# flydog-sdr/FlyDog_SDR_GPS

Hardware: AMD Instinct MI355X
Metric: IQ Msamples/s ingested (waterfall + GPS acq); value = GPS acq, BASELINE configs[1] (higher is better)
Workload: dtype f32

## Files before the change

### flydog_sdr_gps_amd/csrc/kg_acq.hip

```cpp
#include "kg_common.h"
#include "kg_fft.h"

#include <math.h>
#include <stdlib.h>
#include <vector>

#define SUB      4096
#define NTAPS    31
#define DECIM    4


enum { SRC_BITS = 0, SRC_IQ16 = 1, SRC_CHIPS = 2 };

__constant__ float c_hb_even[16] = {
    -0.010233f,  0.010668f, -0.016324f,  0.024377f, -0.036482f,  0.056990f, -0.101993f,
     0.316926f,  0.316926f, -0.101993f,  0.056990f, -0.036482f,  0.024377f, -0.016324f,
     0.010668f, -0.010233f,
};
#define HB_CENTRE 0.500009f

KG_DEV float bipolar(int bit) { return bit ? -1.0f : 1.0f; }

template <int SRC>
KG_DEV cf acq_source(const void *__restrict__ src, int i, int nvalid, int nchips, int boc)
{
    if (i >= nvalid) return cf{0.f, 0.f};
    if constexpr (SRC == SRC_BITS) {
        const uint8_t *p = (const uint8_t *) src;
        const int bit = (p[i >> 3] >> (i & 7)) & 1;
        const int ph = i & 3;
        const int ls = ph < 2, lc = (ph == 0) | (ph == 3);
        return cf{bipolar(bit ^ ls), bipolar(bit ^ lc)};
    } else if constexpr (SRC == SRC_IQ16) {
        const short2 v = ((const short2 *) src)[i];
// ... 134 lines not shown
            if (ii >= 512 - halo) {
                const int jj = (j + 1) & 7;
                kg_st(&o[(jj >> 1) * row + 2 * (ii - 512 + halo) + (jj & 1)], fq[q]);
            }
        }
    }
}

struct acq_red { float p; int i; float s; int pad; };

#define ACQ_CLAIM_STRIDE 32
#define ACQ_LDS_BYTES (2 * SUB * sizeof(float2) + 4 * sizeof(acq_red) + 16)

struct acq_pair_desc {
    int data_off;
    int code_off;
    int limit;
    int out;
};

struct acq_cell_desc { int data_off, code_off, dop, limit, out; };

struct acq_walk {
    int npairs;
    int ndop, dop_lo;
};

template <int P, bool STAMPS = false>
__global__ __launch_bounds__(256, 2) void acq_correlate_kernel(
    const float2 *__restrict__ data,
    const float2 *__restrict__ code,
    const float2 *__restrict__ tab4096, const float2 *__restrict__ tabN,
    const float2 *__restrict__ comb,
    const float2 *__restrict__ quart,
    const acq_pair_desc *__restrict__ pairs,
    int *__restrict__ claim,
    acq_walk walk,
    int halo,
    kg_acq_cell *__restrict__ cells,
    unsigned long long *__restrict__ stamps = nullptr)
{
    static_assert(P == 4 || P == 16, "N = 16384 or 65536");
    constexpr int LOGP = P == 4 ? 2 : 4;
    extern __shared__ __attribute__((aligned(16))) float2 smem[];
    float2 *tileA = smem, *tileB = smem + SUB;
    acq_red *red = (acq_red *) (smem + 2 * SUB);
    volatile int *red_claim = (volatile int *) (red + 4);
    const int t = threadIdx.x;
    unsigned long long *st = (STAMPS && t == 0 && blockIdx.x == 8) ? stamps : nullptr;
    if (STAMPS && st) { st[0] = __builtin_amdgcn_s_memtime(); st[1] = __builtin_amdgcn_s_memrealtime(); }
    unsigned long long *wgt = (STAMPS && t == 0) ? stamps + 512 + 4 * blockIdx.x : nullptr;
    int wg_cells = 0;
    if (STAMPS && wgt) {
        wgt[0] = __builtin_amdgcn_s_memrealtime();
        wgt[2] = (unsigned long long) __builtin_amdgcn_s_getreg((20 << 0) | (0 << 6) | (31 << 11));
    }

    kg_tw4096 tw;
    kg_tw4096_load(tw, tab4096, t);
    cf wb[3], wa[3];
#pragma unroll
    for (int i = 1; i < 4; i++) { wb[i - 1] = kg_ld(&tabN[t * i]); wa[i - 1] = kg_ld(&tabN[(4 * t * i) & (P * SUB - 1)]); }
    (void) wa;
    auto sel3 = [](const cf (&w)[3], int i) { return i == 1 ? w[0] : (i == 2 ? w[1] : w[2]); };

    const int xcd = blockIdx.x & 7, slot = blockIdx.x >> 3, nslots = gridDim.x >> 3;
    const int gpairs = (walk.npairs - xcd + 7) >> 3;
    const bool spread = walk.npairs < 8;
    const int ndop = walk.ndop, ncell = spread ? (walk.npairs * ndop - xcd + 7) >> 3 : gpairs * ndop;

    typedef unsigned u4 __attribute__((ext_vector_type(4)));
    const int rowb_c = 2 * (256 + 2 * halo) * (int) sizeof(float2);
    const int plane_c = 8 * 2 * (256 + 2 * halo);
    cf d[16], c[16];
    struct acq_rsrc { __amdgpu_buffer_rsrc_t drs, crs; int dvo, cvo; };
    auto fetch_prepare = [&](int data_off, int code_off, int dop, int k2) {
        const int s = k2 - dop;
        const int q0 = s >> LOGP;
        acq_rsrc r;
        r.drs = __builtin_amdgcn_make_buffer_rsrc(
            (void *) (data + data_off + k2 * SUB), 0, SUB * (int) sizeof(float2), 0x00020000);
        r.crs = __builtin_amdgcn_make_buffer_rsrc(
            (void *) (code + code_off + (s & (P - 1)) * plane_c), 0, plane_c * (int) sizeof(float2), 0x00020000);
        r.dvo = t * 16; r.cvo = (t + q0 + halo) * 16;
        return r;
    };
    auto fetch_row = [&](const acq_rsrc &r, int i) {
        const u4 dv = __builtin_amdgcn_raw_buffer_load_b128(r.drs, r.dvo, i * 4096, 0);
        const u4 cv = __builtin_amdgcn_raw_buffer_load_b128(r.crs, r.cvo, i * rowb_c, 0);
        d[2 * i] = cf{__uint_as_float(dv[0]), __uint_as_float(dv[1])};
        d[2 * i + 1] = cf{__uint_as_float(dv[2]), __uint_as_float(dv[3])};
        c[2 * i] = cf{__uint_as_float(cv[0]), __uint_as_float(cv[1])};
        c[2 * i + 1] = cf{__uint_as_float(cv[2]), __uint_as_float(cv[3])};
    };
    auto fetch_drow = [&](const acq_rsrc &r, int i) {
        const u4 dv = __builtin_amdgcn_raw_buffer_load_b128(r.drs, r.dvo, i * 4096, 0);
        d[2 * i] = cf{__uint_as_float(dv[0]), __uint_as_float(dv[1])};
        d[2 * i + 1] = cf{__uint_as_float(dv[2]), __uint_as_float(dv[3])};
    };
    auto fetch_crow = [&](const acq_rsrc &r, int i) {
        const u4 cv = __builtin_amdgcn_raw_buffer_load_b128(r.crs, r.cvo, i * rowb_c, 0);
        c[2 * i] = cf{__uint_as_float(cv[0]), __uint_as_float(cv[1])};
        c[2 * i + 1] = cf{__uint_as_float(cv[2]), __uint_as_float(cv[3])};
    };
    auto fetch = [&](int data_off, int code_off, int dop, int k2) {
        const acq_rsrc r = fetch_prepare(data_off, code_off, dop, k2);
#pragma unroll
        for (int i = 0; i < 8; i++) fetch_row(r, i);
    };
    auto describe = [&](int idx) {
        const int cell = spread ? (idx << 3) + xcd : idx;
        const int pg = cell / ndop, di = cell - pg * ndop;
        const acq_pair_desc pd = pairs[spread ? pg : (pg << 3) + xcd];
        return acq_cell_desc{pd.data_off, pd.code_off, walk.dop_lo + di, pd.limit, pd.out + di};
    };

    int cur_idx = slot, nxt_idx = slot + nslots;
    if (cur_idx >= ncell) return;
    acq_cell_desc cur = describe(cur_idx);
    fetch(cur.data_off, cur.code_off, cur.dop, 0);

    int st_item = 0;
    for (;;) {
        const bool more = nxt_idx < ncell;
        const acq_cell_desc nxt = describe(more ? nxt_idx : cur_idx);
        int claimed = 0;
        if (t == 0) claimed = __hip_atomic_fetch_add(&claim[xcd * ACQ_CLAIM_STRIDE], 1, __ATOMIC_RELAXED, __HIP_MEMORY_SCOPE_AGENT);
        cf acc[16];
        cf yprev[16], pbase = cf{0.f, 0.f}, pg[3], pG[3];
        auto accumulate = [&](const cf (&yv)[16], int kp, cf bs, const cf (&g)[3], const cf (&G)[3]) {
            if (kp == 0) {
#pragma unroll
                for (int m = 0; m < 16; m++) acc[m] = yv[m];
                return;
            }
            cf B1, B2, B3;
            kg_cmul1x3s(B1, B2, B3, bs, G[0], G[1], G[2]);
#pragma unroll
            for (int a = 0; a < 4; a++) {
                const cf Ba = a == 0 ? bs : (a == 1 ? B1 : (a == 2 ? B2 : B3));
                const cf C0 = Ba;
                cf C1, C2, C3;
                kg_cmul1x3s(C1, C2, C3, Ba, g[0], g[1], g[2]);
                kg_cmac4v(acc[4 * a], acc[4 * a + 1], acc[4 * a + 2], acc[4 * a + 3],
                          yv[4 * a], yv[4 * a + 1], yv[4 * a + 2], yv[4 * a + 3], C0, C1, C2, C3);
            }
        };
        auto accumulate_fenced = [&](int kp) { kg_pin(); accumulate(yprev, kp, pbase, pg, pG); kg_pin(); };
        const int tl = t & 15, th = t >> 4;
        const int rd = t ^ (th & 15);
#pragma unroll 1
        for (int k2 = 0; k2 < P; k2++) {
            unsigned long long *sti = (STAMPS && st && st_item < 24) ? st + 16 + 16 * st_item : nullptr;
            KG_STAMP(STAMPS, sti, 8);
            cf base;
            if constexpr (P == 4) base = sel3(wb, k2);
            else {
                const int ka = k2 >> 2, kb = k2 & 3;
                const cf A = sel3(wa, ka), Bv = sel3(wb, kb);
                base = ka == 0 ? Bv : (kb == 0 ? A : kg_cmul(A, Bv));
            }
            cf x[16], y[16];
            const bool same = k2 < P - 1;
            const acq_rsrc nr = fetch_prepare(same ? cur.data_off : nxt.data_off, same ? cur.code_off : nxt.code_off,
                                              same ? cur.dop : nxt.dop, (k2 + 1) & (P - 1));
            KG_STAMP(STAMPS, sti, 9);
            KG_STAMP(STAMPS, sti, 10);
            kg_cc_radix16_h<+1>(c, d, y, [&](int s) {
                kg_pin();
                if (s < 4) {
                    fetch_drow(nr, 2 * s); fetch_drow(nr, 2 * s + 1);
                } else {
#pragma unroll
                    for (int m = s - 4; m < 16; m += 4) kg_st_tile(&tileA[16 * t + (m ^ tl)], y[m]);
                }
                kg_pin();
            });
            KG_STAMP(STAMPS, sti, 0);
            KG_STAMP(STAMPS, sti, 1);
            __syncthreads();
            KG_STAMP(STAMPS, sti, 2);
#pragma unroll
            for (int j = 0; j < 16; j++) x[j] = kg_ld_tile(&tileA[rd + 256 * j]);
            if (k2 > 0) accumulate_fenced(k2 - 1);
            if (STAMPS) asm volatile("s_waitcnt lgkmcnt(0)" ::: "memory");
            KG_STAMP(STAMPS, sti, 3);
            kg_tw_radix16_h<+1>(x, y, tw.p1, [&](int s) {
                if (s >= 4) {
                    kg_pin();
#pragma unroll
                    for (int m = s - 4; m < 16; m += 4) kg_st_tile(&tileB[t + 16 * (15 * th + m)], y[m]);
                    kg_pin();
                }
            });
            KG_STAMP(STAMPS, sti, 4);
            __syncthreads();
            KG_STAMP(STAMPS, sti, 5);
            cf g[3], G[3];
#pragma unroll
            for (int i = 0; i < 3; i++) { g[i] = kg_ld(&comb[8 * k2 + i]); G[i] = kg_ld(&comb[8 * k2 + 3 + i]); }
#pragma unroll
            for (int j = 0; j < 16; j++) x[j] = kg_ld_tile(&tileB[t + 256 * j]);
            if (STAMPS) asm volatile("s_waitcnt lgkmcnt(0)" ::: "memory");
            KG_STAMP(STAMPS, sti, 6);
            kg_tw_radix16_h<+1>(x, yprev, tw.p2, [&](int s) {
                if (s < 4) { kg_pin(); fetch_crow(nr, 2 * s); fetch_crow(nr, 2 * s + 1); kg_pin(); }
            });
            pbase = base;
#pragma unroll
            for (int i = 0; i < 3; i++) { pg[i] = g[i]; pG[i] = G[i]; }
            KG_STAMP(STAMPS, sti, 7);
            KG_STAMP(STAMPS, sti, 11);
            if (STAMPS) st_item++;
        }
        accumulate(yprev, P - 1, pbase, pg, pG);

        const int limit = cur.limit, full_rows = limit >> 8;
        float bp = 0.f, sum = 0.f;
        int bi = 0;
        if constexpr (P == 4) {
            float pw[16];
#pragma unroll
            for (int m = 0; m < 16; m++) {
                const cf sq = acc[m] * acc[m];
                pw[m] = sq.x + sq.y;
                if (m >= full_rows) {
                    asm volatile("");
                    pw[m] = (t + 256 * m < limit) ? pw[m] : 0.f;
                }
            }
            cf s2 = cf{0.f, 0.f};
#pragma unroll
            for (int m = 0; m < 16; m += 2) s2 = s2 + cf{pw[m], pw[m + 1]};
            sum = s2.x + s2.y;
#pragma unroll
            for (int m = 0; m < 16; m += 2) bp = __builtin_fmaxf(bp, __builtin_fmaxf(pw[m], pw[m + 1]));
            unsigned qm[2] = {0, 0};
#pragma unroll
            for (int m = 7; m >= 0; m -= 2) {
                unsigned long long k0, k1, k2, k3;
                asm("v_cmp_eq_f32_e64 %2, %6, %10\n\tv_cmp_eq_f32_e64 %3, %7, %10\n\t"
                    "v_cmp_eq_f32_e64 %4, %8, %10\n\tv_cmp_eq_f32_e64 %5, %9, %10\n\t"
                    "v_addc_co_u32_e64 %0, %2, %0, %0, %2\n\tv_addc_co_u32_e64 %1, %3, %1, %1, %3\n\t"
                    "v_addc_co_u32_e64 %0, %4, %0, %0, %4\n\tv_addc_co_u32_e64 %1, %5, %1, %1, %5"
                    : "+v"(qm[0]), "+v"(qm[1]), "=&s"(k0), "=&s"(k1), "=&s"(k2), "=&s"(k3)
                    : "v"(pw[m]), "v"(pw[m + 8]), "v"(pw[m - 1]), "v"(pw[m + 7]), "v"(bp));
            }
            const unsigned rowmask = qm[0] | (qm[1] << 8);
// ... 459 lines not shown
    const int t = blockIdx.x * blockDim.x + threadIdx.x;
    if (t >= P * H) return;
    const int k2 = t % P, k1 = t / P;
    const float2 v = src ? src[(size_t) k2 * plane_len(H, layout_src) + plane_pos(k1, 0, H, layout_src)] : make_float2(0.f, 0.f);
    const int T = layout_dst == 0 ? 256 : 512, J = SUB / T;
    dst[(size_t) k2 * plane_len(H, layout_dst) + plane_pos(k1 + T * (J - 1), T, H, layout_dst)] = v;
}

static void to_planes(const float *nat, std::vector<float2> &pl, int P, int H, int layout)
{
    const size_t plane = plane_len(H, layout);
    const int T = layout == 0 ? 256 : 512, J = SUB / T;
    pl.assign(spec_len(P, H), make_float2(0.f, 0.f));
    for (int k = 0; k < P * SUB; k++) {
        const float2 v = make_float2(nat[2 * k], nat[2 * k + 1]);
        const int k1 = k / P, t = k1 & (T - 1), j = k1 / T;
        float2 *p = pl.data() + (size_t) (k % P) * plane;
        p[plane_pos(k1, 0, H, layout)] = v;
        if (t < H) p[plane_pos(t + T * ((j - 1) & (J - 1)), T, H, layout)] = v;
        if (t >= T - H) p[plane_pos(t + T * ((j + 1) & (J - 1)), -T, H, layout)] = v;
    }
}
static void from_planes(const std::vector<float2> &pl, float *nat, int P, int H, int layout)
{
    const size_t plane = plane_len(H, layout);
    for (int k = 0; k < P * SUB; k++) {
        const float2 v = pl[(size_t) (k % P) * plane + plane_pos(k / P, 0, H, layout)];
        nat[2 * k] = v.x; nat[2 * k + 1] = v.y;
    }
}

static float2 unit_root(long k, long n)
{
    k %= n;
    if (k < 0) k += n;
    if (k == 0) return make_float2(1.f, 0.f);
    if (4 * k == n) return make_float2(0.f, 1.f);
    if (2 * k == n) return make_float2(-1.f, 0.f);
    if (4 * k == 3 * n) return make_float2(0.f, -1.f);
    const double a = 2.0 * M_PI * (double) k / (double) n;
    return make_float2((float) cos(a), (float) sin(a));
}

template <int SRC>
static int launch_frontend(kg_acq *a, hipStream_t st, const uint8_t *d_src, size_t stride, int nbatch,
                           int nvalid, int nchips, int boc, float2 *d_td, float2 *d_scratch,
                           float2 *d_planes, float2 *d_planes_b, size_t planes_stride, int halo)
{
    kg_ctx *c = a->ctx;
    hipLaunchKernelGGL(acq_frontend_kernel<SRC>, dim3(a->fft_len / FE_TILE, nbatch), dim3(256), 0,
                       st, d_src, stride, nvalid, nchips, boc, d_td, a->fft_len);
    KG_HIP(hipGetLastError());
    hipLaunchKernelGGL(acq_fft_sub_kernel<false>, dim3(a->P, nbatch), dim3(256), 2 * SUB * sizeof(float2),
                       st, (const float2 *) d_td, d_scratch, (const float2 *) c->d_tab4096, a->P,
                       (unsigned long long *) nullptr);
    KG_HIP(hipGetLastError());
    if (a->P == 4)
        hipLaunchKernelGGL(acq_fft_combine_kernel<4>, dim3(SUB / 256, nbatch), dim3(256), 0, st,
                           (const float2 *) d_scratch, d_planes, d_planes_b, planes_stride,
                           (const float2 *) a->d_tabN, halo);
    else
        hipLaunchKernelGGL(acq_fft_combine_kernel<16>, dim3(SUB / 256, nbatch), dim3(256), 0, st,
                           (const float2 *) d_scratch, d_planes, d_planes_b, planes_stride,
                           (const float2 *) a->d_tabN, halo);
    KG_HIP(hipGetLastError());
    return KG_OK;
}

static int acq_init(kg_acq *a)
{
    kg_ctx *ctx = a->ctx;
    const int max_sats = a->max_sats, max_blocks = a->max_blocks, N = a->fft_len, P = a->P;
    {
        const int m = (a->dop_hi > -a->dop_lo ? a->dop_hi : -a->dop_lo);
        a->halo = (m + P - 1) / P + 2;
        a->code_len = spec_len(P, a->halo);
    }
    a->limits.assign(max_sats, 0); a->code_set.assign(max_sats, 0); a->code_layout.assign(max_sats, 0);
    a->last_first = a->last_nblocks = a->last_nsats = a->np1 = a->np4 = a->table_nblocks = 0;
    a->d_pairs1 = a->d_pairs4 = nullptr; a->pairs_seq = 0;
    a->in_stride = (size_t) a->nsamples * 4;
    const size_t spec = sizeof(float2) * N;
    if (N == 16384) { a->d_tabN = ctx->d_tab16384; a->own_tabN = false; }
    else {
        std::vector<float2> h(N);
        for (int k = 0; k < N; k++) h[k] = unit_root(k, N);
        KG_HIP(hipMalloc((void **) &a->d_tabN, spec));
        a->own_tabN = true;
        KG_HIP(hipMemcpy(a->d_tabN, h.data(), spec, hipMemcpyHostToDevice));
    }
    {
        const long R = N / 256;
        std::vector<float2> comb(P * 8, make_float2(1.f, 0.f)), quart(P * 4);
        static const int mult[6] = {1, 2, 3, 4, 8, 12};
        for (int k2 = 0; k2 < P; k2++) {
            for (int i = 0; i < 6; i++) comb[8 * k2 + i] = unit_root((long) mult[i] * k2, R);
            for (int q = 0; q < 4; q++) quart[4 * k2 + q] = unit_root((long) q * k2, P);
        }
        KG_HIP(hipMalloc((void **) &a->d_comb, sizeof(float2) * comb.size()));
        KG_HIP(hipMalloc((void **) &a->d_quart, sizeof(float2) * quart.size()));
        KG_HIP(hipMemcpy(a->d_comb, comb.data(), sizeof(float2) * comb.size(), hipMemcpyHostToDevice));
        KG_HIP(hipMemcpy(a->d_quart, quart.data(), sizeof(float2) * quart.size(), hipMemcpyHostToDevice));
        std::vector<float2> comb8(P * 4);
        for (int k2 = 0; k2 < P; k2++)
            for (int k = 0; k < 4; k++) comb8[4 * k2 + k] = unit_root((long) (k + 1) * k2, N / 512);
        KG_HIP(hipMalloc((void **) &a->d_comb8, sizeof(float2) * comb8.size()));
        KG_HIP(hipMemcpy(a->d_comb8, comb8.data(), sizeof(float2) * comb8.size(), hipMemcpyHostToDevice));
    }
    KG_HIP(hipMalloc((void **) &a->d_code, sizeof(float2) * a->code_len * max_sats));
    KG_HIP(hipMalloc((void **) &a->d_data, spec * max_blocks));
    KG_HIP(hipMalloc((void **) &a->d_td, spec * max_blocks));
    KG_HIP(hipMalloc((void **) &a->d_td_code, spec));
    KG_HIP(hipMalloc((void **) &a->d_fsub, spec * max_blocks));
    KG_HIP(hipMalloc((void **) &a->d_fsub_code, spec));
    KG_HIP(hipMalloc((void **) &a->d_in, a->in_stride * max_blocks));
    for (int k = 0; k < 4; k++) {
        KG_HIP(hipHostMalloc((void **) &a->h_pin[k], a->in_stride, hipHostMallocDefault));
        KG_HIP(hipEventCreateWithFlags(&a->ev_pin[k], hipEventDisableTiming));
    }
    KG_HIP(hipEventCreateWithFlags(&a->ev_batch, hipEventDisableTiming));
    KG_HIP(hipEventCreateWithFlags(&a->ev_in_free, hipEventDisableTiming));
    { const int rc_ = kg_stream_get(ctx->device, &a->cstream); if (rc_) return rc_; }
    KG_HIP(hipMalloc((void **) &a->d_chips, 8192));
    KG_HIP(hipMalloc((void **) &a->d_cells, sizeof(kg_acq_cell) * (size_t) max_blocks * max_sats * a->ndop));
    KG_HIP(hipMalloc((void **) &a->d_results, sizeof(kg_acq_result) * (size_t) max_blocks * max_sats));
    KG_HIP(hipMalloc((void **) &a->d_claim, sizeof(int) * 16 * ACQ_CLAIM_STRIDE));
    KG_HIP(hipMemset(a->d_claim, 0, sizeof(int) * 16 * ACQ_CLAIM_STRIDE));
    {
        const char *e = kg_tuning_env("KIWIGPU_ACQ_FRONT_STREAM");
        if (e && e[0] == '1') {
            { const int rc_ = kg_stream_get(ctx->device, &a->fstream); if (rc_) return rc_; }
// ... 393 lines not shown
    KG_HIP(hipStreamSynchronize(a->fstream));
    return KG_OK;
}

int kg_acq_get_data_fft(kg_acq *a, int block, float *data_fft)
{
    int rc = check_block(a, block, data_fft, "kg_acq_get_data_fft");
    if (rc) return rc;
    return get_planes(a, a->d_data + (size_t) block * a->fft_len, data_fft, 0, 0);
}

int kg_acq_get_data_td(kg_acq *a, int block, float *td)
{
    int rc = check_block(a, block, td, "kg_acq_get_data_td");
    if (rc) return rc;
    KG_HIP(hipStreamSynchronize(a->fstream));
    KG_HIP(hipMemcpyAsync(td, a->d_td + (size_t) block * a->fft_len, sizeof(float2) * a->fft_len,
                          hipMemcpyDeviceToHost, a->ctx->stream));
    KG_HIP(hipStreamSynchronize(a->ctx->stream));
    return KG_OK;
}

}

template <int P, bool STAMPS>
static void launch_correlate(kg_acq *a, hipStream_t st, int first, const acq_pair_desc *d_pairs, int npairs,
                             unsigned long long *d_stamps)
{
    const int grid = a->grid1;
    const acq_walk w = {npairs, a->ndop, a->dop_lo};
    hipLaunchKernelGGL((acq_correlate_kernel<P, STAMPS>), dim3(grid), dim3(256), ACQ_LDS_BYTES, st,
                       (const float2 *) (a->d_data + (size_t) first * a->fft_len), (const float2 *) a->d_code,
                       (const float2 *) a->ctx->d_tab4096, (const float2 *) a->d_tabN,
                       (const float2 *) a->d_comb, (const float2 *) a->d_quart, d_pairs,
                       a->d_claim, w, a->halo, a->d_cells, d_stamps);
}

extern "C" {

int kg_acq_correlate_blocks_async(kg_acq *a, int first, int nblocks, const int *sats, int nsats)
{
    KG_REQUIRE(a && sats, KG_ERR_INVALID, "kg_acq_correlate_async: null argument");
    int rc = kg_ctx_use(a->ctx);
    if (rc) return rc;
    KG_REQUIRE(nblocks >= 1 && first >= 0 && first + nblocks <= a->max_blocks, KG_ERR_INVALID,
               "kg_acq_correlate_async: blocks %d..%d (max %d)", first, first + nblocks - 1,
               a->max_blocks);
    KG_REQUIRE(nsats >= 1 && nsats <= a->max_sats, KG_ERR_INVALID,
               "kg_acq_correlate_async: nsats %d (max %d)", nsats, a->max_sats);
    hipStream_t st = a->ctx->stream;
    bool same = (int) a->last_sats.size() == nsats && a->table_nblocks == nblocks &&
                a->ctx->ring_next - a->pairs_seq < KG_RING_SLOTS / 2;
    for (int i = 0; same && i < nsats; i++) same = a->last_sats[i] == sats[i];
    if (!same) {
        for (int i = 0; i < nsats; i++) {
            KG_REQUIRE(sats[i] >= 0 && sats[i] < a->max_sats, KG_ERR_INVALID,
                       "kg_acq_correlate_async: sats[%d] = %d out of range", i, sats[i]);
            KG_REQUIRE(a->code_set[sats[i]], KG_ERR_STATE,
                       "kg_acq_correlate_async: no code set for sat %d", sats[i]);
        }
        std::vector<acq_pair_desc> tab[2];
        for (int blk = 0; blk < nblocks; blk++)
            for (int i = 0; i < nsats; i++) {
                const int sat = sats[i];
                acq_pair_desc pd;
                pd.data_off = blk * a->fft_len;
                pd.code_off = (int) (sat * a->code_len);
// ... 161 lines not shown
```

### flydog_sdr_gps_amd/csrc/kg_fft.h

```cpp
#pragma once

#include <hip/hip_runtime.h>
#include "kg_tables.h"

typedef float cf __attribute__((ext_vector_type(2)));

#define KG_DEV __device__ __forceinline__

KG_DEV cf kg_scale(cf a, float s) { return a * cf{s, s}; }
KG_DEV cf kg_ld(const float2 *p) { return *reinterpret_cast<const cf *>(p); }
KG_DEV void kg_st(float2 *p, cf v) { *reinterpret_cast<cf *>(p) = v; }
KG_DEV cf kg_ld_tile(const float2 *p) { return *(const volatile cf __attribute__((address_space(3))) *) p; }
KG_DEV void kg_st_tile(float2 *p, cf v) { *(volatile cf __attribute__((address_space(3))) *) p = v; }

KG_DEV cf kg_cmul(cf a, cf w)
{
    cf r, d;
    asm("v_pk_mul_f32 %0, %1, %2 op_sel_hi:[1,0]" : "=v"(r) : "v"(a), "v"(w));
    asm("v_pk_fma_f32 %0, %1, %2, %3 op_sel:[1,1,0] op_sel_hi:[0,1,1] neg_lo:[0,1,0]"
        : "=v"(d) : "v"(a), "v"(w), "v"(r));
    return d;
}
KG_DEV cf kg_cmulc(cf a, cf w)
{
    cf r, d;
    asm("v_pk_mul_f32 %0, %1, %2 op_sel_hi:[1,0]" : "=v"(r) : "v"(a), "v"(w));
    asm("v_pk_fma_f32 %0, %1, %2, %3 op_sel:[1,1,0] op_sel_hi:[0,1,1] neg_hi:[0,1,0]"
        : "=v"(d) : "v"(a), "v"(w), "v"(r));
    return d;
}
KG_DEV cf kg_addj(cf a, cf b)
{
    cf d;
    asm("v_pk_add_f32 %0, %1, %2 op_sel:[0,1] op_sel_hi:[1,0] neg_lo:[0,1]" : "=v"(d) : "v"(a), "v"(b));
    return d;
}
KG_DEV cf kg_subj(cf a, cf b)
{
    cf d;
    asm("v_pk_add_f32 %0, %1, %2 op_sel:[0,1] op_sel_hi:[1,0] neg_hi:[0,1]" : "=v"(d) : "v"(a), "v"(b));
    return d;
}
template <int SIGN> KG_DEV cf kg_twmul(cf a, cf w)
{
    return SIGN > 0 ? kg_cmul(a, w) : kg_cmulc(a, w);
}
template <int SIGN> KG_DEV cf kg_sub_sj(cf a, cf b) { return SIGN > 0 ? kg_subj(a, b) : kg_addj(a, b); }

#define KG_MUL_(r, a, w) "v_pk_mul_f32 " r ", " a ", " w " op_sel_hi:[1,0]\n\t"
#define KG_FMA_(a, w, r, neg) "v_pk_fma_f32 " a ", " a ", " w ", " r " op_sel:[1,1,0] op_sel_hi:[0,1,1] " neg "\n\t"

#define KG_FMA3_(o, a, w, neg) "v_pk_fma_f32 " o ", " a ", " w ", " o " op_sel:[1,1,0] op_sel_hi:[0,1,1] " neg "\n\t"
KG_DEV void kg_cmul1x3s(cf &o0, cf &o1, cf &o2, cf a, cf w0, cf w1, cf w2)
{
    asm(KG_MUL_("%0", "%3", "%4") KG_MUL_("%1", "%3", "%5") KG_MUL_("%2", "%3", "%6")
        KG_FMA3_("%0", "%3", "%4", "neg_lo:[0,1,0]") KG_FMA3_("%1", "%3", "%5", "neg_lo:[0,1,0]")
        KG_FMA3_("%2", "%3", "%6", "neg_lo:[0,1,0]")
        : "=&v"(o0), "=&v"(o1), "=&v"(o2) : "v"(a), "s"(w0), "s"(w1), "s"(w2));
}

KG_DEV void kg_cmul1x3v(cf &o0, cf &o1, cf &o2, cf a, cf w0, cf w1, cf w2)
{
    asm(KG_MUL_("%0", "%3", "%4") KG_MUL_("%1", "%3", "%5") KG_MUL_("%2", "%3", "%6")
        KG_FMA3_("%0", "%3", "%4", "neg_lo:[0,1,0]") KG_FMA3_("%1", "%3", "%5", "neg_lo:[0,1,0]")
        KG_FMA3_("%2", "%3", "%6", "neg_lo:[0,1,0]")
        : "=&v"(o0), "=&v"(o1), "=&v"(o2) : "v"(a), "v"(w0), "v"(w1), "v"(w2));
}

template <bool CONJ> KG_DEV void kg_cmul4v(cf &a0, cf &a1, cf &a2, cf &a3, cf w0, cf w1, cf w2, cf w3)
{
    cf r0, r1, r2, r3;
    if constexpr (!CONJ)
        asm(KG_MUL_("%4", "%0", "%8") KG_MUL_("%5", "%1", "%9") KG_MUL_("%6", "%2", "%10") KG_MUL_("%7", "%3", "%11")
            KG_FMA_("%0", "%8", "%4", "neg_lo:[0,1,0]") KG_FMA_("%1", "%9", "%5", "neg_lo:[0,1,0]")
            KG_FMA_("%2", "%10", "%6", "neg_lo:[0,1,0]") KG_FMA_("%3", "%11", "%7", "neg_lo:[0,1,0]")
            : "+v"(a0), "+v"(a1), "+v"(a2), "+v"(a3), "=&v"(r0), "=&v"(r1), "=&v"(r2), "=&v"(r3)
            : "v"(w0), "v"(w1), "v"(w2), "v"(w3));
    else
        asm(KG_MUL_("%4", "%0", "%8") KG_MUL_("%5", "%1", "%9") KG_MUL_("%6", "%2", "%10") KG_MUL_("%7", "%3", "%11")
            KG_FMA_("%0", "%8", "%4", "neg_hi:[0,1,0]") KG_FMA_("%1", "%9", "%5", "neg_hi:[0,1,0]")
            KG_FMA_("%2", "%10", "%6", "neg_hi:[0,1,0]") KG_FMA_("%3", "%11", "%7", "neg_hi:[0,1,0]")
            : "+v"(a0), "+v"(a1), "+v"(a2), "+v"(a3), "=&v"(r0), "=&v"(r1), "=&v"(r2), "=&v"(r3)
            : "v"(w0), "v"(w1), "v"(w2), "v"(w3));
}
template <bool CONJ> KG_DEV void kg_cmul4s(cf &a0, cf &a1, cf &a2, cf &a3, cf w0, cf w1, cf w2, cf w3)
{
    cf r0, r1, r2, r3;
    if constexpr (!CONJ)
        asm(KG_MUL_("%4", "%0", "%8") KG_MUL_("%5", "%1", "%9") KG_MUL_("%6", "%2", "%10") KG_MUL_("%7", "%3", "%11")
            KG_FMA_("%0", "%8", "%4", "neg_lo:[0,1,0]") KG_FMA_("%1", "%9", "%5", "neg_lo:[0,1,0]")
            KG_FMA_("%2", "%10", "%6", "neg_lo:[0,1,0]") KG_FMA_("%3", "%11", "%7", "neg_lo:[0,1,0]")
            : "+v"(a0), "+v"(a1), "+v"(a2), "+v"(a3), "=&v"(r0), "=&v"(r1), "=&v"(r2), "=&v"(r3)
            : "s"(w0), "s"(w1), "s"(w2), "s"(w3));
// ... 3 lines not shown
            KG_FMA_("%2", "%10", "%6", "neg_hi:[0,1,0]") KG_FMA_("%3", "%11", "%7", "neg_hi:[0,1,0]")
            : "+v"(a0), "+v"(a1), "+v"(a2), "+v"(a3), "=&v"(r0), "=&v"(r1), "=&v"(r2), "=&v"(r3)
            : "s"(w0), "s"(w1), "s"(w2), "s"(w3));
}
template <bool CONJ> KG_DEV void kg_cmul3v(cf &a0, cf &a1, cf &a2, cf w0, cf w1, cf w2)
{
    cf r0, r1, r2;
    if constexpr (!CONJ)
        asm(KG_MUL_("%3", "%0", "%6") KG_MUL_("%4", "%1", "%7") KG_MUL_("%5", "%2", "%8")
            KG_FMA_("%0", "%6", "%3", "neg_lo:[0,1,0]") KG_FMA_("%1", "%7", "%4", "neg_lo:[0,1,0]")
            KG_FMA_("%2", "%8", "%5", "neg_lo:[0,1,0]")
            : "+v"(a0), "+v"(a1), "+v"(a2), "=&v"(r0), "=&v"(r1), "=&v"(r2) : "v"(w0), "v"(w1), "v"(w2));
    else
        asm(KG_MUL_("%3", "%0", "%6") KG_MUL_("%4", "%1", "%7") KG_MUL_("%5", "%2", "%8")
            KG_FMA_("%0", "%6", "%3", "neg_hi:[0,1,0]") KG_FMA_("%1", "%7", "%4", "neg_hi:[0,1,0]")
            KG_FMA_("%2", "%8", "%5", "neg_hi:[0,1,0]")
            : "+v"(a0), "+v"(a1), "+v"(a2), "=&v"(r0), "=&v"(r1), "=&v"(r2) : "v"(w0), "v"(w1), "v"(w2));
}
KG_DEV void kg_cmac4v(cf &c0, cf &c1, cf &c2, cf &c3, cf y0, cf y1, cf y2, cf y3, cf w0, cf w1, cf w2, cf w3)
{
#define KG_MAC1_(c, y, w) "v_pk_fma_f32 " c ", " y ", " w ", " c " op_sel_hi:[0,1,1]\n\t"
#define KG_MAC2_(c, y, w) "v_pk_fma_f32 " c ", " y ", " w ", " c " op_sel:[1,1,0] op_sel_hi:[1,0,1] neg_lo:[0,1,0]\n\t"
    asm(KG_MAC1_("%0", "%4", "%8") KG_MAC1_("%1", "%5", "%9") KG_MAC1_("%2", "%6", "%10") KG_MAC1_("%3", "%7", "%11")
        KG_MAC2_("%0", "%4", "%8") KG_MAC2_("%1", "%5", "%9") KG_MAC2_("%2", "%6", "%10") KG_MAC2_("%3", "%7", "%11")
        : "+v"(c0), "+v"(c1), "+v"(c2), "+v"(c3)
        : "v"(y0), "v"(y1), "v"(y2), "v"(y3), "v"(w0), "v"(w1), "v"(w2), "v"(w3));
}
KG_DEV void kg_cmac4v1(cf &c0, cf &c1, cf &c2, cf &c3, cf y0, cf y1, cf y2, cf y3, cf w)
{
    asm(KG_MAC1_("%0", "%4", "%8") KG_MAC1_("%1", "%5", "%8") KG_MAC1_("%2", "%6", "%8") KG_MAC1_("%3", "%7", "%8")
        KG_MAC2_("%0", "%4", "%8") KG_MAC2_("%1", "%5", "%8") KG_MAC2_("%2", "%6", "%8") KG_MAC2_("%3", "%7", "%8")
        : "+v"(c0), "+v"(c1), "+v"(c2), "+v"(c3)
        : "v"(y0), "v"(y1), "v"(y2), "v"(y3), "v"(w));
}
#undef KG_MAC1_
#undef KG_MAC2_

template <int SIGN> KG_DEV void kg_addsub_sj(cf &p, cf &q, cf a, cf b)
{
    if constexpr (SIGN > 0)
        asm("v_pk_add_f32 %0, %2, %3 op_sel:[0,1] op_sel_hi:[1,0] neg_lo:[0,1]\n\t"
            "v_pk_add_f32 %1, %2, %3 op_sel:[0,1] op_sel_hi:[1,0] neg_hi:[0,1]"
            : "=&v"(p), "=v"(q) : "v"(a), "v"(b));
    else
        asm("v_pk_add_f32 %0, %2, %3 op_sel:[0,1] op_sel_hi:[1,0] neg_hi:[0,1]\n\t"
            "v_pk_add_f32 %1, %2, %3 op_sel:[0,1] op_sel_hi:[1,0] neg_lo:[0,1]"
            : "=&v"(p), "=v"(q) : "v"(a), "v"(b));
}
template <int SIGN, bool X2J = false> KG_DEV void kg_radix4(cf &x0, cf &x1, cf &x2, cf &x3)
{
    cf s02, d02;
    if constexpr (X2J) kg_addsub_sj<SIGN>(s02, d02, x0, x2);
    else { s02 = x0 + x2; d02 = x0 - x2; }
    const cf s13 = x1 + x3, d13 = x1 - x3;
    x0 = s02 + s13;
    x2 = s02 - s13;
    kg_addsub_sj<SIGN>(x1, x3, d02, d13);
}

template <int SIGN> KG_DEV void kg_radix16(cf (&x)[16], cf (&y)[16])
{
#pragma unroll
    for (int b = 0; b < 4; b++) kg_radix4<SIGN>(x[b], x[4 + b], x[8 + b], x[12 + b]);
#define KG_W16C(K) cf{KG_W16[K][0], KG_W16[K][1]}
    kg_cmul4s<(SIGN < 0)>(x[5], x[6], x[7], x[9], KG_W16C(1), KG_W16C(2), KG_W16C(3), KG_W16C(2));
    kg_cmul4s<(SIGN < 0)>(x[11], x[13], x[14], x[15], KG_W16C(6), KG_W16C(3), KG_W16C(6), KG_W16C(9));
// ... 69 lines not shown
    } else {
        asm(KG_MUL_("%0", "%3", "%6") KG_MUL_("%1", "%4", "%7") KG_MUL_("%2", "%5", "%8")
            KG_CFMA2C_("%0", "%3", "%6") KG_CFMA2C_("%1", "%4", "%7") KG_CFMA2C_("%2", "%5", "%8")
            : "=&v"(u1[0]), "=&v"(u1[1]), "=&v"(u1[2]) : "v"(x[5]), "v"(x[9]), "v"(x[13]), "s"(KG_W16C(1)), "s"(KG_W16C(2)), "s"(KG_W16C(3)));
        asm(KG_CFMA1_("%0", "%6", "%9", "%3") KG_CFMA1_("%1", "%7", "%10", "%4") KG_CFMA1_("%2", "%8", "%11", "%5")
            KG_CFMA2C_("%0", "%6", "%9") KG_CFMA2C_("%1", "%7", "%10") KG_CFMA2C_("%2", "%8", "%11")
            : "=&v"(s13[0]), "=&v"(s13[1]), "=&v"(s13[2])
            : "v"(u1[0]), "v"(u1[1]), "v"(u1[2]), "v"(x[7]), "v"(x[11]), "v"(x[15]), "s"(KG_W16C(3)), "s"(KG_W16C(6)), "s"(KG_W16C(9)));
        asm(KG_CFMA1_("%0", "%4", "%6", "%2") KG_CFMA1_("%1", "%5", "%7", "%3")
            KG_CFMA2C_("%0", "%4", "%6") KG_CFMA2C_("%1", "%5", "%7")
            : "=&v"(s02a), "=&v"(s02b) : "v"(x[4]), "v"(x[12]), "v"(x[6]), "v"(x[14]), "s"(KG_W16C(2)), "s"(KG_W16C(6)));
    }
    asm(KG_2CMT_("%0", "%5", "%15", "%10") KG_2CMT_("%1", "%6", "%15", "%11") KG_2CMT_("%2", "%7", "%15", "%12")
        KG_2CMT_("%3", "%8", "%15", "%13") KG_2CMT_("%4", "%9", "%15", "%14")
        : "=&v"(d13[0]), "=&v"(d13[1]), "=&v"(d13[2]), "=&v"(d02a), "=&v"(d02b)
        : "v"(u1[0]), "v"(u1[1]), "v"(u1[2]), "v"(x[4]), "v"(x[12]),
          "v"(s13[0]), "v"(s13[1]), "v"(s13[2]), "v"(s02a), "v"(s02b), "s"(two));
    y[1] = s02a + s13[0]; y[9] = s02a - s13[0];
    kg_addsub_sj<SIGN>(y[5], y[13], d02a, d13[0]);
    hook(5);
    {
        cf s02, d02;
        kg_addsub_sj<SIGN>(s02, d02, x[8], x[10]);
        y[2] = s02 + s13[1]; y[10] = s02 - s13[1];
        kg_addsub_sj<SIGN>(y[6], y[14], d02, d13[1]);
    }
    hook(6);
    y[3] = s02b + s13[2]; y[11] = s02b - s13[2];
    kg_addsub_sj<SIGN>(y[7], y[15], d02b, d13[2]);
    hook(7);
#undef KG_W16C
}

template <int SIGN, class H> KG_DEV void kg_radix16_stage1_tw(cf (&x)[16], const kg_tw15 &w, H hook)
{
    constexpr bool CJ = SIGN < 0;
    kg_cmul3v<CJ>(x[1], x[2], x[3], w.w[0], w.w[1], w.w[2]);
    hook(0);
    kg_cmul4v<CJ>(x[4], x[5], x[6], x[7], w.w[3], w.w[4], w.w[5], w.w[6]);
    hook(1);
    cf s02[4], s13[4];
    kg_cfma4v<CJ>(s02[0], s02[1], s02[2], s02[3], x[0], x[1], x[2], x[3], x[8], x[9], x[10], x[11], w.w[7], w.w[8], w.w[9], w.w[10]);
    hook(2);
    kg_cfma4v<CJ>(s13[0], s13[1], s13[2], s13[3], x[4], x[5], x[6], x[7], x[12], x[13], x[14], x[15], w.w[11], w.w[12], w.w[13], w.w[14]);
    hook(3);
    cf d02[4], d13[4];
    kg_2cmt4(d02[0], d02[1], d02[2], d02[3], x[0], x[1], x[2], x[3], s02[0], s02[1], s02[2], s02[3]);
    kg_2cmt4(d13[0], d13[1], d13[2], d13[3], x[4], x[5], x[6], x[7], s13[0], s13[1], s13[2], s13[3]);
#pragma unroll
    for (int b = 0; b < 4; b++) {
        x[b] = s02[b] + s13[b];
        x[8 + b] = s02[b] - s13[b];
        kg_addsub_sj<SIGN>(x[4 + b], x[12 + b], d02[b], d13[b]);
    }
}

template <int SIGN, class H> KG_DEV void kg_radix16_stage1_cc(const cf (&c)[16], const cf (&d)[16], cf (&x)[16], H hook)
{
    cf u0[4], u1[4];
    kg_cmul4v_o<true>(u0[0], u0[1], u0[2], u0[3], c[0], c[1], c[2], c[3], d[0], d[1], d[2], d[3]);
    hook(0);
    kg_cmul4v_o<true>(u1[0], u1[1], u1[2], u1[3], c[4], c[5], c[6], c[7], d[4], d[5], d[6], d[7]);
    hook(1);
    cf s02[4], s13[4];
    kg_cfma4v<true>(s02[0], s02[1], s02[2], s02[3], u0[0], u0[1], u0[2], u0[3], c[8], c[9], c[10], c[11], d[8], d[9], d[10], d[11]);
    hook(2);
    kg_cfma4v<true>(s13[0], s13[1], s13[2], s13[3], u1[0], u1[1], u1[2], u1[3], c[12], c[13], c[14], c[15], d[12], d[13], d[14], d[15]);
    hook(3);
    cf d02[4], d13[4];
    kg_2cmt4(d02[0], d02[1], d02[2], d02[3], u0[0], u0[1], u0[2], u0[3], s02[0], s02[1], s02[2], s02[3]);
    kg_2cmt4(d13[0], d13[1], d13[2], d13[3], u1[0], u1[1], u1[2], u1[3], s13[0], s13[1], s13[2], s13[3]);
#pragma unroll
    for (int b = 0; b < 4; b++) {
        x[b] = s02[b] + s13[b];
        x[8 + b] = s02[b] - s13[b];
        kg_addsub_sj<SIGN>(x[4 + b], x[12 + b], d02[b], d13[b]);
    }
}

#define kg_pin() __builtin_amdgcn_sched_barrier(0)
template <int SIGN, class H> KG_DEV void kg_tw_radix16_h(cf (&x)[16], cf (&y)[16], const kg_tw15 &w, H hook)
{
    kg_radix16_stage1_tw<SIGN>(x, w, hook);
    kg_radix16_stage2f<SIGN>(x, y, hook);
}
template <int SIGN, class H> KG_DEV void kg_cc_radix16_h(const cf (&c)[16], const cf (&d)[16], cf (&y)[16], H hook)
{
    cf x[16];
    kg_radix16_stage1_cc<SIGN>(c, d, x, hook);
    kg_radix16_stage2f<SIGN>(x, y, hook);
}

struct kg_tw4096 { kg_tw15 p1, p2; };

KG_DEV void kg_tw4096_load(kg_tw4096 &tw, const float2 *__restrict__ tab4096, int t)
{
#pragma unroll
    for (int j = 1; j < 16; j++) {
        tw.p1.w[j - 1] = kg_ld(&tab4096[(j * (t & 15)) << 4]);
        tw.p2.w[j - 1] = kg_ld(&tab4096[j * t]);
    }
}

template <int SIGN> KG_DEV void kg_twiddle16(cf (&x)[16], const kg_tw15 &w)
{
    kg_cmul4v<(SIGN < 0)>(x[1], x[2], x[3], x[4], w.w[0], w.w[1], w.w[2], w.w[3]);
    kg_cmul4v<(SIGN < 0)>(x[5], x[6], x[7], x[8], w.w[4], w.w[5], w.w[6], w.w[7]);
    kg_cmul4v<(SIGN < 0)>(x[9], x[10], x[11], x[12], w.w[8], w.w[9], w.w[10], w.w[11]);
    kg_cmul3v<(SIGN < 0)>(x[13], x[14], x[15], w.w[12], w.w[13], w.w[14]);
}

#define KG_STAMP(on, ptr, i)                                                          \
    do {                                                                              \
        if (on) {                                                                     \
            __builtin_amdgcn_sched_barrier(0);                                        \
            if ((ptr) != nullptr) (ptr)[i] = __builtin_amdgcn_s_memtime();            \
            __builtin_amdgcn_sched_barrier(0);                                        \
        }                                                                             \
// ... 243 lines not shown
```

Baseline: 2640.

## Fold row twiddles into last radix-16 stage and accumulate via Horner

Rewrites the cross-k2 accumulation of the acquisition correlator. Per-row twiddle constants are folded into the final radix-16 stage through a new 12-entry scalar table. The outer k2 loop now runs in reverse, so accumulation becomes a Horner recurrence with one per-thread constant per group, replacing per-iteration base/comb complex multiplies. It also forces the data-row offset into an SGPR via inline asm. This removes several complex multiplies and scalar loads per k2 step, at the cost of more SGPR constants in the stage-2 asm and changed rounding order.

After: 2699, median of 6. 2.2% higher.

```diff
diff --git a/flydog_sdr_gps_amd/csrc/kg_acq.hip b/flydog_sdr_gps_amd/csrc/kg_acq.hip
--- a/flydog_sdr_gps_amd/csrc/kg_acq.hip
+++ b/flydog_sdr_gps_amd/csrc/kg_acq.hip
@@ -1,5 +1,6 @@
 #include "kg_common.h"
 #include "kg_fft.h"
+#include "kg_acq_tables.h"
 
 #include <math.h>
 #include <stdlib.h>
@@ -200,7 +201,6 @@
     const float2 *__restrict__ code,
     const float2 *__restrict__ tab4096, const float2 *__restrict__ tabN,
     const float2 *__restrict__ comb,
-    const float2 *__restrict__ quart,
     const acq_pair_desc *__restrict__ pairs,
     int *__restrict__ claim,
     acq_walk walk,
@@ -226,11 +226,9 @@
 
     kg_tw4096 tw;
     kg_tw4096_load(tw, tab4096, t);
-    cf wb[3], wa[3];
-#pragma unroll
-    for (int i = 1; i < 4; i++) { wb[i - 1] = kg_ld(&tabN[t * i]); wa[i - 1] = kg_ld(&tabN[(4 * t * i) & (P * SUB - 1)]); }
-    (void) wa;
-    auto sel3 = [](const cf (&w)[3], int i) { return i == 1 ? w[0] : (i == 2 ? w[1] : w[2]); };
+    cf V[4];
+#pragma unroll
+    for (int dd = 0; dd < 4; dd++) V[dd] = kg_ld(&tabN[t + 1024 * dd]);
 
     const int xcd = blockIdx.x & 7, slot = blockIdx.x >> 3, nslots = gridDim.x >> 3;
     const int gpairs = (walk.npairs - xcd + 7) >> 3;
@@ -262,7 +260,9 @@
         c[2 * i + 1] = cf{__uint_as_float(cv[2]), __uint_as_float(cv[3])};
     };
     auto fetch_drow = [&](const acq_rsrc &r, int i) {
-        const u4 dv = __builtin_amdgcn_raw_buffer_load_b128(r.drs, r.dvo, i * 4096, 0);
+        int so;
+        asm volatile("s_mov_b32 %0, %1" : "=s"(so) : "i"(i * 4096));
+        const u4 dv = __builtin_amdgcn_raw_buffer_load_b128(r.drs, r.dvo, so, 0);
         d[2 * i] = cf{__uint_as_float(dv[0]), __uint_as_float(dv[1])};
         d[2 * i + 1] = cf{__uint_as_float(dv[2]), __uint_as_float(dv[3])};
     };
@@ -286,7 +286,7 @@
     int cur_idx = slot, nxt_idx = slot + nslots;
     if (cur_idx >= ncell) return;
     acq_cell_desc cur = describe(cur_idx);
-    fetch(cur.data_off, cur.code_off, cur.dop, 0);
+    fetch(cur.data_off, cur.code_off, cur.dop, P - 1);
 
     int st_item = 0;
     for (;;) {
@@ -295,43 +295,29 @@
         int claimed = 0;
         if (t == 0) claimed = __hip_atomic_fetch_add(&claim[xcd * ACQ_CLAIM_STRIDE], 1, __ATOMIC_RELAXED, __HIP_MEMORY_SCOPE_AGENT);
         cf acc[16];
-        cf yprev[16], pbase = cf{0.f, 0.f}, pg[3], pG[3];
-        auto accumulate = [&](const cf (&yv)[16], int kp, cf bs, const cf (&g)[3], const cf (&G)[3]) {
-            if (kp == 0) {
+        cf yprev[16];
+        auto accumulate = [&](cf (&yv)[16], bool first) {
+            if (first) {
 #pragma unroll
                 for (int m = 0; m < 16; m++) acc[m] = yv[m];
                 return;
             }
-            cf B1, B2, B3;
-            kg_cmul1x3s(B1, B2, B3, bs, G[0], G[1], G[2]);
-#pragma unroll
-            for (int a = 0; a < 4; a++) {
-                const cf Ba = a == 0 ? bs : (a == 1 ? B1 : (a == 2 ? B2 : B3));
-                const cf C0 = Ba;
-                cf C1, C2, C3;
-                kg_cmul1x3s(C1, C2, C3, Ba, g[0], g[1], g[2]);
-                kg_cmac4v(acc[4 * a], acc[4 * a + 1], acc[4 * a + 2], acc[4 * a + 3],
-                          yv[4 * a], yv[4 * a + 1], yv[4 * a + 2], yv[4 * a + 3], C0, C1, C2, C3);
-            }
+#pragma unroll
+            for (int dd = 0; dd < 4; dd++)
+                kg_horner4v(acc[4 * dd], acc[4 * dd + 1], acc[4 * dd + 2], acc[4 * dd + 3],
+                            yv[4 * dd], yv[4 * dd + 1], yv[4 * dd + 2], yv[4 * dd + 3], V[dd]);
         };
-        auto accumulate_fenced = [&](int kp) { kg_pin(); accumulate(yprev, kp, pbase, pg, pG); kg_pin(); };
+        auto accumulate_fenced = [&](bool first) { kg_pin(); accumulate(yprev, first); kg_pin(); };
         const int tl = t & 15, th = t >> 4;
         const int rd = t ^ (th & 15);
 #pragma unroll 1
-        for (int k2 = 0; k2 < P; k2++) {
+        for (int k2 = P - 1; k2 >= 0; k2--) {
             unsigned long long *sti = (STAMPS && st && st_item < 24) ? st + 16 + 16 * st_item : nullptr;
             KG_STAMP(STAMPS, sti, 8);
-            cf base;
-            if constexpr (P == 4) base = sel3(wb, k2);
-            else {
-                const int ka = k2 >> 2, kb = k2 & 3;
-                const cf A = sel3(wa, ka), Bv = sel3(wb, kb);
-                base = ka == 0 ? Bv : (kb == 0 ? A : kg_cmul(A, Bv));
-            }
             cf x[16], y[16];
-            const bool same = k2 < P - 1;
+            const bool same = k2 > 0;
             const acq_rsrc nr = fetch_prepare(same ? cur.data_off : nxt.data_off, same ? cur.code_off : nxt.code_off,
-                                              same ? cur.dop : nxt.dop, (k2 + 1) & (P - 1));
+                                              same ? cur.dop : nxt.dop, (k2 - 1) & (P - 1));
             KG_STAMP(STAMPS, sti, 9);
             KG_STAMP(STAMPS, sti, 10);
             kg_cc_radix16_h<+1>(c, d, y, [&](int s) {
@@ -350,7 +336,7 @@
             KG_STAMP(STAMPS, sti, 2);
 #pragma unroll
             for (int j = 0; j < 16; j++) x[j] = kg_ld_tile(&tileA[rd + 256 * j]);
-            if (k2 > 0) accumulate_fenced(k2 - 1);
+            if (k2 < P - 1) accumulate_fenced(k2 == P - 2);
             if (STAMPS) asm volatile("s_waitcnt lgkmcnt(0)" ::: "memory");
             KG_STAMP(STAMPS, sti, 3);
             kg_tw_radix16_h<+1>(x, y, tw.p1, [&](int s) {
@@ -364,24 +350,21 @@
             KG_STAMP(STAMPS, sti, 4);
             __syncthreads();
             KG_STAMP(STAMPS, sti, 5);
-            cf g[3], G[3];
-#pragma unroll
-            for (int i = 0; i < 3; i++) { g[i] = kg_ld(&comb[8 * k2 + i]); G[i] = kg_ld(&comb[8 * k2 + 3 + i]); }
+            cf rk[KG_ACQ_ROWK];
+#pragma unroll
+            for (int i = 0; i < KG_ACQ_ROWK; i++) rk[i] = kg_ld(&comb[KG_ACQ_ROWK * k2 + i]);
 #pragma unroll
             for (int j = 0; j < 16; j++) x[j] = kg_ld_tile(&tileB[t + 256 * j]);
             if (STAMPS) asm volatile("s_waitcnt lgkmcnt(0)" ::: "memory");
             KG_STAMP(STAMPS, sti, 6);
-            kg_tw_radix16_h<+1>(x, yprev, tw.p2, [&](int s) {
+            kg_tw_radix16_hk<+1>(x, yprev, tw.p2, rk, [&](int s) {
                 if (s < 4) { kg_pin(); fetch_crow(nr, 2 * s); fetch_crow(nr, 2 * s + 1); kg_pin(); }
             });
-            pbase = base;
-#pragma unroll
-            for (int i = 0; i < 3; i++) { pg[i] = g[i]; pG[i] = G[i]; }
             KG_STAMP(STAMPS, sti, 7);
             KG_STAMP(STAMPS, sti, 11);
             if (STAMPS) st_item++;
         }
-        accumulate(yprev, P - 1, pbase, pg, pG);
+        accumulate(yprev, false);
 
         const int limit = cur.limit, full_rows = limit >> 8;
         float bp = 0.f, sum = 0.f;
@@ -907,14 +890,9 @@
 
 static float2 unit_root(long k, long n)
 {
-    k %= n;
-    if (k < 0) k += n;
-    if (k == 0) return make_float2(1.f, 0.f);
-    if (4 * k == n) return make_float2(0.f, 1.f);
-    if (2 * k == n) return make_float2(-1.f, 0.f);
-    if (4 * k == 3 * n) return make_float2(0.f, -1.f);
-    const double a = 2.0 * M_PI * (double) k / (double) n;
-    return make_float2((float) cos(a), (float) sin(a));
+    float2 r;
+    kg_unit_root_f(k, n, &r.x, &r.y);
+    return r;
 }
 
 template <int SRC>
@@ -965,13 +943,11 @@
         KG_HIP(hipMemcpy(a->d_tabN, h.data(), spec, hipMemcpyHostToDevice));
     }
     {
-        const long R = N / 256;
-        std::vector<float2> comb(P * 8, make_float2(1.f, 0.f)), quart(P * 4);
-        static const int mult[6] = {1, 2, 3, 4, 8, 12};
-        for (int k2 = 0; k2 < P; k2++) {
-            for (int i = 0; i < 6; i++) comb[8 * k2 + i] = unit_root((long) mult[i] * k2, R);
+        std::vector<float2> comb(P * KG_ACQ_ROWK), quart(P * 4);
+        static_assert(sizeof(float2) == 2 * sizeof(float), "float2 = (re, im)");
+        kg_acq_row_consts(P, &comb[0].x);
+        for (int k2 = 0; k2 < P; k2++)
             for (int q = 0; q < 4; q++) quart[4 * k2 + q] = unit_root((long) q * k2, P);
-        }
         KG_HIP(hipMalloc((void **) &a->d_comb, sizeof(float2) * comb.size()));
         KG_HIP(hipMalloc((void **) &a->d_quart, sizeof(float2) * quart.size()));
         KG_HIP(hipMemcpy(a->d_comb, comb.data(), sizeof(float2) * comb.size(), hipMemcpyHostToDevice));
@@ -1431,7 +1407,7 @@
     hipLaunchKernelGGL((acq_correlate_kernel<P, STAMPS>), dim3(grid), dim3(256), ACQ_LDS_BYTES, st,
                        (const float2 *) (a->d_data + (size_t) first * a->fft_len), (const float2 *) a->d_code,
                        (const float2 *) a->ctx->d_tab4096, (const float2 *) a->d_tabN,
-                       (const float2 *) a->d_comb, (const float2 *) a->d_quart, d_pairs,
+                       (const float2 *) a->d_comb, d_pairs,
                        a->d_claim, w, a->halo, a->d_cells, d_stamps);
 }
 
diff --git a/flydog_sdr_gps_amd/csrc/kg_acq_tables.h b/flydog_sdr_gps_amd/csrc/kg_acq_tables.h
--- /dev/null
+++ b/flydog_sdr_gps_amd/csrc/kg_acq_tables.h
@@ -0,0 +1,27 @@
+#pragma once
+
+#include <math.h>
+
+static inline void kg_unit_root_f(long k, long n, float *re, float *im)
+{
+    k %= n;
+    if (k < 0) k += n;
+    if (k == 0) { *re = 1.f; *im = 0.f; return; }
+    if (4 * k == n) { *re = 0.f; *im = 1.f; return; }
+    if (2 * k == n) { *re = -1.f; *im = 0.f; return; }
+    if (4 * k == 3 * n) { *re = 0.f; *im = -1.f; return; }
+    const double a = 2.0 * M_PI * (double) k / (double) n;
+    *re = (float) cos(a); *im = (float) sin(a);
+}
+
+#define KG_ACQ_ROWK 12
+static inline void kg_acq_row_consts(int P, float *out)
+{
+    const long R = 16L * P;
+    for (int k2 = 0; k2 < P; k2++)
+        for (int c = 1; c < 4; c++)
+            for (int d = 0; d < 4; d++) {
+                float *o = out + 2 * (KG_ACQ_ROWK * k2 + 4 * (c - 1) + d);
+                kg_unit_root_f((long) c * (d * (R / 16) + k2), R, &o[0], &o[1]);
+            }
+}
diff --git a/flydog_sdr_gps_amd/csrc/kg_fft.h b/flydog_sdr_gps_amd/csrc/kg_fft.h
--- a/flydog_sdr_gps_amd/csrc/kg_fft.h
+++ b/flydog_sdr_gps_amd/csrc/kg_fft.h
@@ -51,14 +51,6 @@
 #define KG_FMA_(a, w, r, neg) "v_pk_fma_f32 " a ", " a ", " w ", " r " op_sel:[1,1,0] op_sel_hi:[0,1,1] " neg "\n\t"
 
 #define KG_FMA3_(o, a, w, neg) "v_pk_fma_f32 " o ", " a ", " w ", " o " op_sel:[1,1,0] op_sel_hi:[0,1,1] " neg "\n\t"
-KG_DEV void kg_cmul1x3s(cf &o0, cf &o1, cf &o2, cf a, cf w0, cf w1, cf w2)
-{
-    asm(KG_MUL_("%0", "%3", "%4") KG_MUL_("%1", "%3", "%5") KG_MUL_("%2", "%3", "%6")
-        KG_FMA3_("%0", "%3", "%4", "neg_lo:[0,1,0]") KG_FMA3_("%1", "%3", "%5", "neg_lo:[0,1,0]")
-        KG_FMA3_("%2", "%3", "%6", "neg_lo:[0,1,0]")
-        : "=&v"(o0), "=&v"(o1), "=&v"(o2) : "v"(a), "s"(w0), "s"(w1), "s"(w2));
-}
-
 KG_DEV void kg_cmul1x3v(cf &o0, cf &o1, cf &o2, cf a, cf w0, cf w1, cf w2)
 {
     asm(KG_MUL_("%0", "%3", "%4") KG_MUL_("%1", "%3", "%5") KG_MUL_("%2", "%3", "%6")
@@ -128,6 +120,15 @@
         KG_MAC2_("%0", "%4", "%8") KG_MAC2_("%1", "%5", "%8") KG_MAC2_("%2", "%6", "%8") KG_MAC2_("%3", "%7", "%8")
         : "+v"(c0), "+v"(c1), "+v"(c2), "+v"(c3)
         : "v"(y0), "v"(y1), "v"(y2), "v"(y3), "v"(w));
+}
+KG_DEV void kg_horner4v(cf &c0, cf &c1, cf &c2, cf &c3, cf &z0, cf &z1, cf &z2, cf &z3, cf v)
+{
+#define KG_HOR2_(c, v, z) "v_pk_fma_f32 " c ", " c ", " v ", " z " op_sel:[1,1,0] op_sel_hi:[1,0,1] neg_lo:[0,1,0]\n\t"
+    asm(KG_MAC1_("%4", "%0", "%8") KG_MAC1_("%5", "%1", "%8") KG_MAC1_("%6", "%2", "%8") KG_MAC1_("%7", "%3", "%8")
+        KG_HOR2_("%0", "%8", "%4") KG_HOR2_("%1", "%8", "%5") KG_HOR2_("%2", "%8", "%6") KG_HOR2_("%3", "%8", "%7")
+        : "+v"(c0), "+v"(c1), "+v"(c2), "+v"(c3), "+v"(z0), "+v"(z1), "+v"(z2), "+v"(z3)
+        : "v"(v));
+#undef KG_HOR2_
 }
 #undef KG_MAC1_
 #undef KG_MAC2_
@@ -263,6 +264,45 @@
 #undef KG_W16C
 }
 
+template <int SIGN, class H> KG_DEV void kg_radix16_stage2f_k(cf (&x)[16], cf (&y)[16], const cf (&k)[12], H hook)
+{
+    const cf two = cf{2.0f, 2.0f};
+    kg_radix4<SIGN>(x[0], x[1], x[2], x[3]);
+    y[0] = x[0]; y[4] = x[1]; y[8] = x[2]; y[12] = x[3];
+    hook(4);
+    cf u0[3], u1[3], s02[3], s13[3], d02[3], d13[3];
+#define KG_S2K_PRODUCTS_(F2)                                                                                                     \
+    asm(KG_MUL_("%0", "%6", "%12") KG_MUL_("%1", "%7", "%13") KG_MUL_("%2", "%8", "%14")                                           \
+        KG_MUL_("%3", "%9", "%15") KG_MUL_("%4", "%10", "%16") KG_MUL_("%5", "%11", "%17")                                         \
+        F2("%0", "%6", "%12") F2("%1", "%7", "%13") F2("%2", "%8", "%14") F2("%3", "%9", "%15") F2("%4", "%10", "%16") F2("%5", "%11", "%17") \
+        : "=&v"(u0[0]), "=&v"(u0[1]), "=&v"(u0[2]), "=&v"(u1[0]), "=&v"(u1[1]), "=&v"(u1[2])                                     \
+        : "v"(x[4]), "v"(x[8]), "v"(x[12]), "v"(x[5]), "v"(x[9]), "v"(x[13]),                                                   \
+          "s"(k[0]), "s"(k[4]), "s"(k[8]), "s"(k[1]), "s"(k[5]), "s"(k[9]))
+#define KG_S2K_SUMS_(F2)                                                                                                         \
+    asm(KG_CFMA1_("%0", "%12", "%18", "%6") KG_CFMA1_("%1", "%13", "%19", "%7") KG_CFMA1_("%2", "%14", "%20", "%8")              \
+        KG_CFMA1_("%3", "%15", "%21", "%9") KG_CFMA1_("%4", "%16", "%22", "%10") KG_CFMA1_("%5", "%17", "%23", "%11")            \
+        F2("%0", "%12", "%18") F2("%1", "%13", "%19") F2("%2", "%14", "%20") F2("%3", "%15", "%21") F2("%4", "%16", "%22") F2("%5", "%17", "%23") \
+        : "=&v"(s02[0]), "=&v"(s02[1]), "=&v"(s02[2]), "=&v"(s13[0]), "=&v"(s13[1]), "=&v"(s13[2])                               \
+        : "v"(u0[0]), "v"(u0[1]), "v"(u0[2]), "v"(u1[0]), "v"(u1[1]), "v"(u1[2]),                                               \
+          "v"(x[6]), "v"(x[10]), "v"(x[14]), "v"(x[7]), "v"(x[11]), "v"(x[15]),                                                 \
+          "s"(k[2]), "s"(k[6]), "s"(k[10]), "s"(k[3]), "s"(k[7]), "s"(k[11]))
+    if constexpr (SIGN > 0) { KG_S2K_PRODUCTS_(KG_CFMA2P_); KG_S2K_SUMS_(KG_CFMA2P_); }
+    else { KG_S2K_PRODUCTS_(KG_CFMA2C_); KG_S2K_SUMS_(KG_CFMA2C_); }
+#undef KG_S2K_PRODUCTS_
+#undef KG_S2K_SUMS_
+    asm(KG_2CMT_("%0", "%6", "%18", "%12") KG_2CMT_("%1", "%7", "%18", "%13") KG_2CMT_("%2", "%8", "%18", "%14")
+        KG_2CMT_("%3", "%9", "%18", "%15") KG_2CMT_("%4", "%10", "%18", "%16") KG_2CMT_("%5", "%11", "%18", "%17")
+        : "=&v"(d02[0]), "=&v"(d02[1]), "=&v"(d02[2]), "=&v"(d13[0]), "=&v"(d13[1]), "=&v"(d13[2])
+        : "v"(u0[0]), "v"(u0[1]), "v"(u0[2]), "v"(u1[0]), "v"(u1[1]), "v"(u1[2]),
+          "v"(s02[0]), "v"(s02[1]), "v"(s02[2]), "v"(s13[0]), "v"(s13[1]), "v"(s13[2]), "s"(two));
+#pragma unroll
+    for (int c = 1; c < 4; c++) {
+        y[c] = s02[c - 1] + s13[c - 1]; y[c + 8] = s02[c - 1] - s13[c - 1];
+        kg_addsub_sj<SIGN>(y[c + 4], y[c + 12], d02[c - 1], d13[c - 1]);
+        hook(4 + c);
+    }
+}
+
 template <int SIGN, class H> KG_DEV void kg_radix16_stage1_tw(cf (&x)[16], const kg_tw15 &w, H hook)
 {
     constexpr bool CJ = SIGN < 0;
@@ -315,6 +355,11 @@
     kg_radix16_stage1_tw<SIGN>(x, w, hook);
     kg_radix16_stage2f<SIGN>(x, y, hook);
 }
+template <int SIGN, class H> KG_DEV void kg_tw_radix16_hk(cf (&x)[16], cf (&y)[16], const kg_tw15 &w, const cf (&k)[12], H hook)
+{
+    kg_radix16_stage1_tw<SIGN>(x, w, hook);
+    kg_radix16_stage2f_k<SIGN>(x, y, k, hook);
+}
 template <int SIGN, class H> KG_DEV void kg_cc_radix16_h(const cf (&c)[16], const cf (&d)[16], cf (&y)[16], H hook)
 {
     cf x[16];
```
